# JunweiLiang/FVTA_MemexQA

Hardware: AMD Instinct MI355X
Metric: QA-pairs/sec (fwd+bwd) at B=64, 40 photos x 5 streams x 30 tok, h=512 (higher is better)
Workload: dtype bf16; 1 GPU; BASELINE.json configs[2] train step (fwd+bwd+adam), shape 'metric', dense lengths; qa_pairs_per_gpu=64, albums=1, photos=40, text_streams=5, hidden=512, global_batch=64, K=6, T=1200, JQ=30, parallelism=dp1 (QA pairs sharded, flat-gradient all-reduce)

## Files before the change

### fvta_memexqa_amd/csrc/lstm.hip

```cpp
#include "gemm_f32.h"
#include "fvta_prof.h"
#include <vector>

#include "lstm_common.h"

namespace fvta {

__device__ const float k_ones4[4] = {1.f, 0.f, 0.f, 0.f};


__global__ __launch_bounds__(1024) void plan_sort_kernel(PlanView v, const int32_t* __restrict__ len_in,
                                                         const int32_t* __restrict__ seq_J_in,
                                                         const int64_t* __restrict__ x_off_in,
                                                         const int64_t* __restrict__ out_off_in,
                                                         int64_t out_ld, int B, int J, int in, int d,
                                                         int64_t x_bw_delta) {
  extern __shared__ int32_t sh[];
  const int tid = threadIdx.x, wave = tid >> 6, lane = tid & 63;
  const int NW = 16, H = J + 1;
  for (int i = tid; i < NW * H; i += 1024) sh[i] = 0;
  const bool fresh = v.hdr->magic != PLAN_MAGIC || v.hdr->B != B || v.hdr->J != J || v.hdr->d != d || v.hdr->out_ld != out_ld;
  __syncthreads();
  if (tid == 0) {
    v.hdr->out_ld = out_ld;
// ... 599 lines not shown
  fvta_prof_end(FVTA_PROF_LSTM_STEP_FWD + 16 * d->reserved, launches, stream);
  FVTA_CHECK_LAUNCH("lstm_step_fwd");
  return FVTA_OK;
}

extern "C" int fvta_bilstm_bwd(const fvta_lstm_desc* d, const void* plan, const float* x, const float* out,
                               const float* d_out, const float* kernel_fw, const float* kernel_bw, void* saved,
                               float* dx, float* dkernel_fw, float* dbias_fw, float* dkernel_bw,
                               float* dbias_bw, void* workspace, fvta_stream_t stream_) {
  return fvta_bilstm_bwd_hint(d, plan, x, out, d_out, kernel_fw, kernel_bw, saved, dx, dkernel_fw, dbias_fw, dkernel_bw,
                              dbias_bw, workspace, stream_, nullptr, nullptr);
}

extern "C" int fvta_bilstm_bwd_overlap(const fvta_lstm_desc* d, const void* plan, const float* x, const float* out,
                                       const float* d_out, const float* kernel_fw, const float* kernel_bw, void* saved,
                                       float* dx, float* dkernel_fw, float* dbias_fw, float* dkernel_bw,
                                       float* dbias_bw, void* workspace, fvta_stream_t stream_,
                                       fvta_stream_t side_stream_) {
  return fvta_bilstm_bwd_hint(d, plan, x, out, d_out, kernel_fw, kernel_bw, saved, dx, dkernel_fw, dbias_fw, dkernel_bw,
                              dbias_bw, workspace, stream_, side_stream_, nullptr);
}

extern "C" int fvta_bilstm_bwd_hint(const fvta_lstm_desc* d, const void* plan, const float* x, const float* out,
                                    const float* d_out, const float* kernel_fw, const float* kernel_bw, void* saved,
                                    float* dx, float* dkernel_fw, float* dbias_fw, float* dkernel_bw,
                                    float* dbias_bw, void* workspace, fvta_stream_t stream_,
                                    fvta_stream_t side_stream_, const int32_t* nactive_host) {
  if (int e = check_lstm_desc(d)) return e;
  FVTA_CHECK_ARG(d->training, "bilstm_bwd: forward was not run with training=1");
  FVTA_CHECK_ARG(plan && x && out && d_out && kernel_fw && saved && dkernel_fw && dbias_fw && workspace,
                 "bilstm_bwd: null pointer");
  FVTA_CHECK_ARG(d->share_fw_bw || (kernel_bw && dkernel_bw && dbias_bw), "bilstm_bwd: *_bw pointers required");
  hipStream_t stream = (hipStream_t)stream_;
  PlanView pv = plan_view(d, const_cast<void*>(plan));
  SavedView sv = saved_view(d, saved);
  WorkView wv = work_view(d, workspace);
  const int B = d->B, J = d->J, in = d->in, dd = d->d;
  if (!lstm_is_bf(d)) FVTA_CHECK_HIP(hipMemsetAsync(wv.cstate, 0, (size_t)2 * B * dd * sizeof(float) * 2, stream));
  GateBwdArgs g;
  g.plan = pv;
  g.d_out = d_out;
  g.gates = sv.gates;
  g.gatesb = sv.gatesb;
  g.cs = sv.cs;
  g.dc = wv.cstate;
  g.dh_rec = wv.dh_rec;
  const bool bf = lstm_is_bf(d);
  g.dzb = bf ? wv.dzb : nullptr;
  g.B = B;
  g.J = J;
  g.d = dd;
  StepBwdArgs s;
  s.plan = pv;
  s.dz = sv.gates;
  s.W[0] = kernel_fw;
  s.W[1] = d->share_fw_bw ? kernel_fw : kernel_bw;
  s.dx = dx;
  s.dh_rec = wv.dh_rec;
  s.dzb = wv.dzb;
  s.in_i = in_internal(d);
  const int dbg = fvta_diag_env("FVTA_DEBUG_SKIP", 0);
  s.dbg = dbg;
  s.Wb[0] = wv.wb[0];
  s.Wb[1] = d->share_fw_bw ? wv.wb[0] : wv.wb[1];
  s.B = B;
  s.J = J;
  s.in = in;
  s.d = dd;
  const dim3 ggrid((unsigned)(((size_t)B * dd + 255) / 256), 1, 2);
  const dim3 sgrid((B + MmaSq::BM - 1) / MmaSq::BM, (in + dd + MmaSq::BN - 1) / MmaSq::BN, 2);
  const size_t sh = MmaSq::LDS_FLOATS * sizeof(float);
  DwArgs w;
  w.plan = pv;
  w.x = x;
  w.out = out;
  w.dz = sv.gates;
  w.slabs = wv.slabs;
  w.B = B;
  w.J = J;
  w.in = in;
  w.d = dd;
  w.tgroup = dw_tgroup(d);
  w.nsplit = dw_nsplit(d);
  w.dzb = wv.dzb;
  w.in_i = in_internal(d);
  w.xs = sv.xs;
  w.hs = sv.hs;
  w.xm = lstm_xm(d);
  (void)side_stream_;
  fvta_prof_begin(FVTA_PROF_LSTM_STEP_BWD + 16 * d->reserved, stream);
  if (bf) {
    FusedBwdArgs f;
    f.plan = pv;
    f.Wb[0] = wv.wb[0];
    f.Wb[1] = d->share_fw_bw ? wv.wb[0] : wv.wb[1];
    f.gatesb = sv.gatesb;
    f.cs = sv.cs;
    f.d_out = d_out;
    f.dzb = wv.dzb;
    f.dc = wv.cstate;
    f.dx = dx;
    f.B = B;
    f.J = J;
    f.in = in;
    f.d = dd;
    f.in_i = in_internal(d);
    f.gates32 = sv.gates;
    f.xm = lstm_xm(d);
    f.dx_accumulate = 1;
    f.dx_both = 0;
    if (dx && d->dx_overwrite) {
      const bool direct = dx_writes_whole_rows(f);
      hipLaunchKernelGGL(dx_zero_rows_kernel, dim3((B + 3) / 4), dim3(256), 0, stream, pv, dx, in, direct ? 1 : 0, B);
      f.dx_accumulate = direct ? 0 : 1;
    }
    for (int t = J - 1; t >= 0; --t) {
      f.t = t;
      f.nact_hint = nactive_host ? nactive_host[t] : -1;
      launch_bwd_fused_bf16(f, stream);
    }
    fvta_prof_end(FVTA_PROF_LSTM_STEP_BWD + 16 * d->reserved, J, stream);
    if (dx) {
      fvta_prof_begin(FVTA_PROF_LSTM_DX + 16 * d->reserved, stream);
      launch_dx_bf16(f, stream);
      fvta_prof_end(FVTA_PROF_LSTM_DX + 16 * d->reserved, 1, stream);
    }
  } else {
  if (dx && d->dx_overwrite) hipLaunchKernelGGL(dx_zero_rows_kernel, dim3((B + 3) / 4), dim3(256), 0, stream, pv, dx, in, 0, B);
  for (int t = J - 1; t >= 0; --t) {
    g.t = t;
    s.t = t;
    if (!(dbg & 512)) hipLaunchKernelGGL(lstm_gate_bwd, ggrid, dim3(256), 0, stream, g);
    if (t > 0 || dx) hipLaunchKernelGGL(lstm_step_bwd_f32, sgrid, dim3(256), sh, stream, s);
  }
  }
  if (!bf) fvta_prof_end(FVTA_PROF_LSTM_STEP_BWD + 16 * d->reserved, 2 * J, stream);
  FVTA_CHECK_LAUNCH("lstm_step_bwd");
  const int MM = in + dd + 1, N4 = 4 * dd;
  const dim3 wgrid((MM + MmaSq::BM - 1) / MmaSq::BM, N4 / MmaSq::BN, 2 * w.nsplit);
  fvta_prof_begin(FVTA_PROF_LSTM_DW + 16 * d->reserved, stream);
  if (dbg & 1024) {
  } else if (bf)
    launch_dw_bf16(w, stream);
  else
    hipLaunchKernelGGL(lstm_dw_f32, wgrid, dim3(256), sh, stream, w);
  FVTA_CHECK_LAUNCH("lstm_dw");
  const size_t slab_elems = bf ? (size_t)kpad8(d) * N4 : (size_t)MM * N4;
  const unsigned rgrid = (unsigned)((slab_elems + 255) / 256);
  if (bf) {
    const int ndir = d->share_fw_bw ? 1 : 2;
    for (int i = 0; i < ndir; ++i)
      launch_dw_reduce_bf16(wv.slabs + (size_t)i * w.nsplit * slab_elems, d->share_fw_bw ? 2 * w.nsplit : w.nsplit,
                            in, in_internal(d), dd, i == 0 ? dkernel_fw : dkernel_bw, i == 0 ? dbias_fw : dbias_bw,
                            stream);
  } else if (d->share_fw_bw) {
    hipLaunchKernelGGL(lstm_dw_reduce, dim3(rgrid), dim3(256), 0, stream, wv.slabs, 2 * w.nsplit, slab_elems,
                       in + dd, N4, dkernel_fw, dbias_fw);
  } else {
    hipLaunchKernelGGL(lstm_dw_reduce, dim3(rgrid), dim3(256), 0, stream, wv.slabs, w.nsplit, slab_elems, in + dd,
                       N4, dkernel_fw, dbias_fw);
    hipLaunchKernelGGL(lstm_dw_reduce, dim3(rgrid), dim3(256), 0, stream, wv.slabs + (size_t)w.nsplit * slab_elems,
                       w.nsplit, slab_elems, in + dd, N4, dkernel_bw, dbias_bw);
  }
  fvta_prof_end(FVTA_PROF_LSTM_DW + 16 * d->reserved, 1, stream);
  FVTA_CHECK_LAUNCH("lstm_dw_reduce");
  return FVTA_OK;
// ... 98 lines not shown
```

### fvta_memexqa_amd/csrc/lstm_bf16.hip

```cpp
#include "gemm_bf16.h"
#include "lstm_common.h"

namespace fvta {

__device__ __forceinline__ int il32(int e) { return ((e >> 5) << 6) + (e & 31); }
__global__ void cvt_weights_kernel(const float* __restrict__ W, bf16_t* __restrict__ wt, bf16_t* __restrict__ wb,
                                   int in, int in_i, int d, int xm) {
  __shared__ float tile[32][33];
  const int N4 = 4 * d, Ki = in_i + d;
  const int k0 = blockIdx.y * 32, n0 = blockIdx.x * 32;
  const int tx = threadIdx.x & 31, ty = threadIdx.x >> 5;
  for (int r = ty; r < 32; r += 8) {
    const int k = k0 + r, n = n0 + tx;
    const int src = k < in ? k : (k >= in_i ? in + (k - in_i) : -1);
    const float v = src >= 0 ? W[(size_t)src * N4 + n] : 0.f;
    tile[r][tx] = v;
    const int c = 4 * (n % d) + n / d;
    const bf16_t hi = f2bf(v);
    bf16_t* row = wb + (size_t)k * N4 * xm;
    if (xm == 1) {
      row[c] = hi;
    } else {
      row[il32(c)] = hi;
      row[il32(c) + 32] = f2bf(v - bf2f(hi));
// ... 462 lines not shown
        }
      }
#pragma unroll
      for (int it = 0; it < 4; ++it) {
        const f32x4 v = old[it] + plane_row16(pl, it * 8 + io_row, io_c4);
        if (ok[it] && (!(abl & 4) || v[0] == 1234.5f)) {
          if ((reinterpret_cast<uintptr_t>(ptr[it]) & 15) == 0) {
            *reinterpret_cast<f32x4*>(ptr[it]) = v;
          } else {
            ptr[it][0] = v[0]; ptr[it][1] = v[1]; ptr[it][2] = v[2]; ptr[it][3] = v[3];
          }
        }
      }
      wave_sync();
    }
}

#ifndef FVTA_DX_WIDE
#define FVTA_DX_WIDE 1
#endif
#ifndef FVTA_DX_BOTH
#define FVTA_DX_BOTH 1
#endif
static bool dx_wide_both(const FusedBwdArgs& a) {
  return FVTA_DX_WIDE && FVTA_DX_BOTH && a.in > 128 && a.in <= 256 && (4 * a.d * a.xm) % 64 == 0 &&
         (size_t)a.J * a.B * (4 * a.d * a.xm) * 2 < ((size_t)1 << 32);
}
bool dx_writes_whole_rows(const FusedBwdArgs& a) { return dx_wide_both(a); }

template <int WN, int BK, int ST, bool BOTH, bool NOACC, int XM, int WM = 4, int TN = 4>
static void launch_dx_tile(const FusedBwdArgs& a, dim3 grid, int dir, int accumulate, hipStream_t s) {
  typedef TileCfgT<WN, 2, WM, ST, BK, TN> Cfg;
  auto* k = lstm_dx_bf16<WN, BK, ST, BOTH, NOACC, XM, WM, TN>;
  lstm_launch(k, grid, dim3(Cfg::NT), Cfg::LDS_BYTES + Cfg::BM * 8, s, a, dir, accumulate);
}

template <int XM>
static void launch_dx_xm(const FusedBwdArgs& a, hipStream_t s) {
  if (FVTA_DX_WIDE && a.in > 128 && a.in <= 256 && (4 * a.d * a.xm) % 64 == 0) {
#ifndef FVTA_DX_BK
#define FVTA_DX_BK 64
#define FVTA_DX_ST 2
#endif
    static_assert(XM == 1 || FVTA_DX_BK == 64, "split engine: 64-element stage rows");
    constexpr int BK = FVTA_DX_BK, ST = FVTA_DX_ST;
    const dim3 grid(pad8((a.B + 255) / 256), 1, a.J);
    if (dx_wide_both(a)) {
      FusedBwdArgs b = a;
      b.dx_both = 1;
      if (!a.dx_accumulate)
        launch_dx_tile<2, BK, ST, true, true, XM>(b, grid, 0, 0, s);
      else
        launch_dx_tile<2, BK, ST, true, false, XM>(b, grid, 0, a.dx_accumulate, s);
      launch_dx_tile<2, BK, ST, false, false, XM>(b, grid, 1, a.dx_accumulate, s);
      return;
    }
    for (int dir = 0; dir < 2; ++dir) launch_dx_tile<2, BK, ST, false, false, XM>(a, grid, dir, a.dx_accumulate || dir, s);
    return;
  }
  constexpr int NBK = XM == 1 ? 32 : 64, NST = XM == 1 ? 3 : 2;
  if (XM == 2 && a.B <= 64 && a.in <= 128) {
    const dim3 gridp((a.B + 63) / 64, 1, a.J);
    for (int dir = 0; dir < 2; ++dir) launch_dx_tile<4, NBK, NST, false, false, XM, 1, 1>(a, gridp, dir, a.dx_accumulate || dir, s);
    return;
  }
  const dim3 grid(pad8((a.B + 255) / 256), (a.in + 127) / 128, a.J);
  for (int dir = 0; dir < 2; ++dir) launch_dx_tile<1, NBK, NST, false, false, XM>(a, grid, dir, a.dx_accumulate || dir, s);
}

void launch_dx_bf16(const FusedBwdArgs& a, hipStream_t s) {
  if (a.xm == 2)
    launch_dx_xm<2>(a, s);
  else
    launch_dx_xm<1>(a, s);
}

#ifndef FVTA_DW_STAGES
#define FVTA_DW_STAGES 4
#endif
constexpr int dw_stages(int wn) { return wn == 2 ? FVTA_DW_STAGES : 3; }
template <int WN>
using DwCfg = TileCfgT<WN, 2, 4, dw_stages(WN)>;

template <int WN>
__global__ __launch_bounds__((TileCfgT<WN>::NT), (WN == 1 ? 2 : 1)) void lstm_dw_bf16(DwArgs a) {
  typedef DwCfg<WN> TileCfg;
  typedef MmaBT<WN, 2, 4, dw_stages(WN)> MmaB;
  extern __shared__ __attribute__((aligned(16))) bf16_t smem_h[];
  const int tid = threadIdx.x;
  const int d = a.d, in_i = a.in_i, N4 = 4 * d;
  const int xtiles = (in_i + TileCfg::BM - 1) / TileCfg::BM;
  const int mtiles = xtiles + (d + TileCfg::BM - 1) / TileCfg::BM, ntiles = N4 / TileCfg::BN, per = mtiles * ntiles;
  const int xcd = blockIdx.x & 7, slot = blockIdx.x >> 3;
  const int bz = xcd + 8 * (slot / per);
  const int tile_id = slot % per;
  if (bz >= 2 * a.nsplit) return;
  const int bx = tile_id % mtiles, by = tile_id / mtiles;
  const bool isx = bx < xtiles;
  const int col0 = isx ? bx * TileCfg::BM : (bx - xtiles) * TileCfg::BM;
  const int ncols = isx ? in_i : d;
  const int n0 = by * TileCfg::BN;
  const int split = bz % a.nsplit, dir = bz / a.nsplit;
  MmaB mma;
  mma.init(tid);
  KMajorSrc<TileCfg::BM, TileCfg::A_GLDS> sa;
  KMajorSrc<TileCfg::BN, TileCfg::B_GLDS> sb;
  sa.setup(mma.wave_all, mma.lane, col0, ncols, (unsigned)ncols * 2);
  sb.setup(mma.wave_all, mma.lane, n0, N4, (unsigned)N4 * 2);
  const int t_begin = split * a.tgroup, t_end = min(a.J, t_begin + a.tgroup);
  for (int t = t_begin; t < t_end; ++t) {
    const int nact = a.plan.nactive[t];
    if (nact == 0) break;
    if (!isx && t == 0) continue;
    const size_t trow = ((size_t)dir * a.J + t) * a.B;
    const bf16_t* A = isx ? a.xs + trow * in_i : a.hs + (trow - (size_t)a.B) * d;
    const __amdgpu_buffer_rsrc_t ra = make_rsrc(A, (unsigned)nact * ncols * 2);
    const __amdgpu_buffer_rsrc_t rz = make_rsrc(a.dzb + trow * (size_t)N4, (unsigned)nact * N4 * 2);
    auto issue = [&](int tile, bf16_t* As, bf16_t* Bs) {
      sa.issue(ra, As, mma.wave_all, (unsigned)tile * 32u * ncols * 2u);
      sb.issue(rz, Bs, mma.wave_all, (unsigned)tile * 32u * N4 * 2u);
    };
    glds_mainloop<true>(mma, issue, (nact + 31) / 32, smem_h);
    __builtin_amdgcn_s_barrier();
  }
  float* slab = a.slabs + (size_t)bz * (in_i + d) * N4;
  const int mrow0 = isx ? col0 : in_i + col0;
#pragma unroll
  for (int ti = 0; ti < MmaB::TM; ++ti)
#pragma unroll
    for (int r = 0; r < 16; ++r) {
      const int ml = mma.row_of(ti, r);
      if (col0 + ml >= ncols) continue;
#pragma unroll
      for (int tj = 0; tj < MmaB::TN; ++tj) slab[(size_t)(mrow0 + ml) * N4 + n0 + mma.col_of(tj)] = mma.acc[ti][tj][r];
    }
}

__global__ __launch_bounds__(512, 1) void lstm_dw_x2(DwArgs a) {
  typedef DwX2Cfg TileCfg;
  extern __shared__ __attribute__((aligned(16))) bf16_t smem_h[];
  const int tid = threadIdx.x;
  const int d = a.d, in_i = a.in_i, N4 = 4 * d;
  const int xtiles = (in_i + TileCfg::BM - 1) / TileCfg::BM;
  const int mtiles = xtiles + (d + TileCfg::BM - 1) / TileCfg::BM, ntiles = (N4 + TileCfg::BN - 1) / TileCfg::BN, per = mtiles * ntiles;
  const int xcd = blockIdx.x & 7, slot = blockIdx.x >> 3;
  const int bz = xcd + 8 * (slot / per);
  const int tile_id = slot % per;
  if (bz >= 2 * a.nsplit) return;
  const int bx = tile_id % mtiles, by = tile_id / mtiles;
  const bool isx = bx < xtiles;
  const int col0 = isx ? bx * TileCfg::BM : (bx - xtiles) * TileCfg::BM;
  const int ncols = isx ? in_i : d;
  const int n0 = by * TileCfg::BN;
  const int split = bz % a.nsplit, dir = bz / a.nsplit;
  MmaX2K mma;
  mma.init(tid);
  KMajorSrc<TileCfg::PCOLS, TileCfg::A_GLDS> sa;
  KMajorSrc<TileCfg::PCOLS, TileCfg::B_GLDS> sb;
  sa.setup(mma.wave_all, mma.lane, 2 * col0, 2 * ncols, (unsigned)ncols * 4);
  sb.setup(mma.wave_all, mma.lane, 2 * n0, 2 * N4, (unsigned)N4 * 4);
  const int t_begin = split * a.tgroup, t_end = min(a.J, t_begin + a.tgroup);
  for (int t = t_begin; t < t_end; ++t) {
    const int nact = a.plan.nactive[t];
    if (nact == 0) break;
    if (!isx && t == 0) continue;
    const size_t trow = ((size_t)dir * a.J + t) * a.B;
    const bf16_t* A = isx ? a.xs + trow * (size_t)(2 * in_i) : a.hs + (trow - (size_t)a.B) * (size_t)(2 * d);
    const __amdgpu_buffer_rsrc_t ra = make_rsrc(A, (unsigned)nact * ncols * 4);
    const __amdgpu_buffer_rsrc_t rz = make_rsrc(a.dzb + trow * (size_t)(2 * N4), (unsigned)nact * N4 * 4);
    auto issue = [&](int tile, bf16_t* As, bf16_t* Bs) {
      sa.issue(ra, As, mma.wave_all, (unsigned)tile * TileCfg::KR * ncols * 4u);
      sb.issue(rz, Bs, mma.wave_all, (unsigned)tile * TileCfg::KR * N4 * 4u);
    };
    glds_mainloop<true>(mma, issue, (nact + TileCfg::KR - 1) / TileCfg::KR, smem_h);
    __builtin_amdgcn_s_barrier();
  }
  float* slab = a.slabs + (size_t)bz * (in_i + d) * N4;
  const int mrow0 = isx ? col0 : in_i + col0;
#pragma unroll
  for (int ti = 0; ti < MmaX2K::TM; ++ti)
#pragma unroll
    for (int r = 0; r < 16; ++r) {
      const int ml = mma.row_of(ti, r);
      if (col0 + ml >= ncols) continue;
#pragma unroll
      for (int tj = 0; tj < MmaX2K::TN; ++tj)
        if (n0 + mma.col_of(tj) < N4) slab[(size_t)(mrow0 + ml) * N4 + n0 + mma.col_of(tj)] = mma.acc[ti][tj][r];
    }
}

template <class Cfg, class K>
static void launch_dw_tiles(K* k, const DwArgs& a, hipStream_t s) {
  const int slices8 = (2 * a.nsplit + 7) / 8;
  const int per = ((a.in_i + 255) / 256 + (a.d + 255) / 256) * ((4 * a.d + Cfg::BN - 1) / Cfg::BN);
  lstm_launch(k, dim3(8 * per * slices8), dim3(Cfg::NT), Cfg::LDS_BYTES, s, a);
}
void launch_dw_bf16(const DwArgs& a, hipStream_t s) {
  if (a.xm == 2)
    launch_dw_tiles<DwX2Cfg>(lstm_dw_x2, a, s);
  else if ((4 * a.d) % 256 == 0)
    launch_dw_tiles<DwCfg<2>>(lstm_dw_bf16<2>, a, s);
  else
    launch_dw_tiles<DwCfg<1>>(lstm_dw_bf16<1>, a, s);
}

__global__ __launch_bounds__(256) void lstm_dw_reduce_bf16(const float* __restrict__ slabs, int nslab, int in, int in_i, int d,
                                                            float* __restrict__ dW, float* __restrict__ dbias) {
  const int N4 = 4 * d;
  const size_t slab_elems = (size_t)(in_i + d) * N4;
  const size_t idx = ((size_t)blockIdx.x * blockDim.x + threadIdx.x) * 4;
  if (idx >= slab_elems) return;
  const int row = (int)(idx / N4), u = (int)(idx % N4) >> 2;
  if (row > in && row < in_i) return;
  f32x4 s = f32x4{0.f, 0.f, 0.f, 0.f};
  int k = 0;
  for (; k + 8 <= nslab; k += 8) {
    f32x4 v[8];
#pragma unroll
    for (int j = 0; j < 8; ++j) v[j] = *reinterpret_cast<const f32x4*>(slabs + (size_t)(k + j) * slab_elems + idx);
#pragma unroll
    for (int j = 0; j < 8; ++j) s += v[j];
  }
  for (; k < nslab; ++k) s += *reinterpret_cast<const f32x4*>(slabs + (size_t)k * slab_elems + idx);
  float* dst = row < in ? dW + (size_t)row * N4 : (row == in ? dbias : dW + (size_t)(in + row - in_i) * N4);
#pragma unroll
  for (int g = 0; g < 4; ++g) dst[g * d + u] += s[g];
}

void launch_dw_reduce_bf16(const float* slabs, int nslab, int in, int in_i, int d, float* dW, float* dbias,
                           hipStream_t s) {
  const size_t n = (size_t)(in_i + d) * d;
  lstm_launch(lstm_dw_reduce_bf16, dim3((unsigned)((n + 255) / 256)), dim3(256), 0, s, slabs, nslab, in, in_i, d, dW, dbias);
}

__global__ void cvt_f32_bf16_kernel(const float* __restrict__ src, bf16_t* __restrict__ dst, size_t n) {
  const size_t i = (size_t)blockIdx.x * blockDim.x + threadIdx.x;
  if (i < n) dst[i] = f2bf(src[i]);
}

template <int LAYOUT>
__global__ __launch_bounds__(256, 2) void test_gemm_bf16_kernel(int M, int N, int K, const bf16_t* __restrict__ A,
                                                                const bf16_t* __restrict__ B, float* __restrict__ C) {
  extern __shared__ __attribute__((aligned(16))) bf16_t smem_h[];
  const int tid = threadIdx.x;
  const int m0 = blockIdx.x * TileCfg::BM, n0 = blockIdx.y * TileCfg::BN;
  MmaB mma;
  mma.init(tid);
  if (LAYOUT == 1) {
    const __amdgpu_buffer_rsrc_t ra = make_rsrc(A, (unsigned)M * K * 2), rb = make_rsrc(B, (unsigned)N * K * 2);
    RowSrc<TileCfg::A_GLDS> sa;
    RowSrc<TileCfg::B_GLDS> sb;
    sa.setup(mma.wave, mma.lane, m0, M, K * 2);
    sb.setup(mma.wave, mma.lane, n0, N, K * 2);
    auto issue = [&](int tile, bf16_t* As, bf16_t* Bs) {
      sa.issue(ra, As, mma.wave, tile * 64);
      sb.issue(rb, Bs, mma.wave, tile * 64);
    };
    glds_mainloop_sp(mma, issue, K / 32, smem_h);
  } else {
    const __amdgpu_buffer_rsrc_t ra = make_rsrc(A, (unsigned)K * M * 2), rb = make_rsrc(B, (unsigned)K * N * 2);
    KMajorSrc<TileCfg::BM, TileCfg::A_GLDS> sa;
    KMajorSrc<TileCfg::BN, TileCfg::B_GLDS> sb;
    sa.setup(mma.wave, mma.lane, m0, M, (unsigned)M * 2);
    sb.setup(mma.wave, mma.lane, n0, N, (unsigned)N * 2);
    auto issue = [&](int tile, bf16_t* As, bf16_t* Bs) {
      sa.issue(ra, As, mma.wave, (unsigned)tile * 32u * M * 2u);
      sb.issue(rb, Bs, mma.wave, (unsigned)tile * 32u * N * 2u);
    };
    glds_mainloop<true>(mma, issue, (K + 31) / 32, smem_h);
  }
#pragma unroll
  for (int ti = 0; ti < MmaB::TM; ++ti)
#pragma unroll
    for (int r = 0; r < 16; ++r) {
      const int m = m0 + mma.row_of(ti, r);
#pragma unroll
      for (int tj = 0; tj < MmaB::TN; ++tj) {
        const int n = n0 + mma.col_of(tj);
        if (m < M && n < N) C[(size_t)m * N + n] = mma.acc[ti][tj][r];
// ... 112 lines not shown
```

### fvta_memexqa_amd/csrc/lstm_common.h

```cpp
#pragma once
#include <type_traits>
#include "fvta_common.h"

namespace fvta {

struct PlanHeader {
  int64_t out_ld;
  int32_t B, J, in, d;
  int64_t x_bw_delta;
  uint32_t magic;
  int32_t pad[7];
};
constexpr uint32_t PLAN_MAGIC = 0x46565441u;

struct PlanView {
  PlanHeader* hdr;
  int32_t* order;
  int32_t* nactive;
  int32_t* len;
  int32_t* seq_J;
  int64_t* x_off;
  int64_t* out_off;
  int64_t* xo;
  int64_t* oo;
  int32_t* dirty;
  int64_t* dirty_out;
  size_t bytes;
};

static inline PlanView plan_view(const fvta_lstm_desc* d, void* p) {
  FvtaCarver c(p);
  PlanView v;
  v.hdr = c.take<PlanHeader>(1);
  v.order = c.take<int32_t>(d->B);
  v.nactive = c.take<int32_t>(d->J + 1);
  v.len = c.take<int32_t>(d->B);
  v.seq_J = c.take<int32_t>(d->B);
  v.x_off = c.take<int64_t>(d->B);
  v.out_off = c.take<int64_t>(d->B);
  v.xo = c.take<int64_t>((size_t)2 * d->J * d->B);
  v.oo = c.take<int64_t>((size_t)2 * d->J * d->B);
  v.dirty = c.take<int32_t>(d->B);
  v.dirty_out = c.take<int64_t>(d->B);
  v.bytes = c.off;
  return v;
}

static inline bool lstm_is_bf(const fvta_lstm_desc* d) { return d->precision == FVTA_BF16 || d->precision == FVTA_BF16X3; }
static inline int lstm_xm(const fvta_lstm_desc* d) { return d->precision == FVTA_BF16X3 ? 2 : 1; }

static inline int in_internal(const fvta_lstm_desc* d) { return (d->in + 1 + 31) / 32 * 32; }

struct SavedView {
  float* gates;
  bf16_t* gatesb;
  float* cs;
  bf16_t* xs;
  bf16_t* hs;
  size_t bytes;
};
static inline SavedView saved_view(const fvta_lstm_desc* d, void* p) {
  FvtaCarver c(p);
  SavedView s;
  s.gates = s.cs = nullptr;
  s.xs = s.hs = s.gatesb = nullptr;
  if (d->training) {
    if (d->precision == FVTA_BF16)
      s.gatesb = c.take<bf16_t>((size_t)2 * d->J * d->B * 4 * d->d);
    else
      s.gates = c.take<float>((size_t)2 * d->J * d->B * 4 * d->d);
    s.cs = c.take<float>((size_t)2 * d->J * d->B * d->d);
  }
  if (lstm_is_bf(d)) {
    s.xs = c.take<bf16_t>((size_t)2 * d->J * d->B * in_internal(d) * lstm_xm(d));
    s.hs = c.take<bf16_t>((size_t)2 * d->J * d->B * d->d * lstm_xm(d));
  }
  s.bytes = c.off < 256 ? 256 : c.off;
  return s;
}

static inline int dw_tgroup(const fvta_lstm_desc* d) {
  int g = (d->J + 15) / 16;
  return g < 1 ? 1 : g;
}
static inline int dw_nsplit(const fvta_lstm_desc* d) { return (d->J + dw_tgroup(d) - 1) / dw_tgroup(d); }
static inline int kpad8(const fvta_lstm_desc* d) { return in_internal(d) + d->d; }

struct WorkView {
  float* cstate;
  float* dh_rec;
  float* slabs;
  bf16_t* wt[2];
  bf16_t* wb[2];
  bf16_t* dzb;
  bf16_t* wf[2];
  size_t bytes;
};
static inline WorkView work_view(const fvta_lstm_desc* d, void* p) {
  FvtaCarver c(p);
  WorkView w;
  w.cstate = c.take<float>((size_t)2 * d->B * d->d);
  w.dh_rec = c.take<float>((size_t)2 * d->B * d->d);
  const size_t slab_rows = lstm_is_bf(d) ? (size_t)kpad8(d) : (size_t)(d->in + d->d + 1);
  w.slabs = c.take<float>((size_t)2 * dw_nsplit(d) * slab_rows * 4 * d->d);
  w.wt[0] = w.wt[1] = w.wb[0] = w.wb[1] = nullptr;
  w.dzb = nullptr;
  w.wf[0] = w.wf[1] = nullptr;
  if (lstm_is_bf(d)) {
    const size_t xm = (size_t)lstm_xm(d);
    for (int i = 0; i < 2; ++i) {
      w.wt[i] = c.take<bf16_t>((size_t)4 * d->d * kpad8(d) * xm);
      w.wb[i] = c.take<bf16_t>((size_t)kpad8(d) * 4 * d->d * xm);
    }
    if (d->training) w.dzb = c.take<bf16_t>((size_t)2 * d->J * d->B * 4 * d->d * xm);
    for (int i = 0; i < 2; ++i) w.wf[i] = c.take<bf16_t>((size_t)4 * d->d * kpad8(d) * xm);
  }
  w.bytes = c.off;
  return w;
}

struct StepArgs {
  PlanView plan;
  const float* x;
  float* out;
  const float* W[2];
  const bf16_t* Wt[2];
  const bf16_t* Wf[2];
  const bf16_t* xs;
  bf16_t* hs;
  const float* bias[2];
  float* gates;
  bf16_t* gatesb;
  float* cs;
  float* cstate;
  int t, B, J, in, d, Kp;
  int dbg;
  int xm;
  int nt;
  int64_t out_skip;
};

struct GateBwdArgs {
  PlanView plan;
  const float* d_out;
  float* gates;
  const bf16_t* gatesb;
  bf16_t* dzb;
  const float* cs;
  float* dc;
  float* dh_rec;
  int t, B, J, d;
};

struct StepBwdArgs {
  PlanView plan;
  const float* dz;
  const bf16_t* dzb;
  const float* W[2];
  const bf16_t* Wb[2];
  float* dx;
  float* dh_rec;
  int t, B, J, in, d, in_i;
  int dbg;
};

struct DwArgs {
  PlanView plan;
  const float* x;
  const float* out;
  const float* dz;
  const bf16_t* dzb;
  const bf16_t* xs;
  const bf16_t* hs;
  float* slabs;
  int B, J, in, d, tgroup, nsplit, in_i;
  int xm;
};

#ifdef __HIPCC__
template <class Mma>
__device__ __forceinline__ void lstm_gate_epilogue(const Mma& mma, const StepArgs& a, int dir, int m0, int u0,
                                                   int nact, size_t trow, const int64_t* s_oo) {
  static_assert(Mma::TN == 4 && Mma::WAVES_N == 1, "wave tile must span the four gate strips");
  const int d = a.d, t = a.t;
  const float* __restrict__ bias = a.bias[dir];
  const int u = u0 + mma.l31;
  const float bi = bias[u], bj = bias[d + u], bf = bias[2 * d + u], bo = bias[3 * d + u];
  const float* cprev_src = a.cs ? a.cs + (trow - a.B) * (size_t)d : a.cstate + (size_t)dir * a.B * d;
#pragma unroll
  for (int ti = 0; ti < Mma::TM; ++ti) {
    float cp[16];
#pragma unroll
    for (int r = 0; r < 16; ++r) {
      const int i = min(m0 + mma.row_of(ti, r), nact - 1);
      cp[r] = (t > 0 && !(a.dbg & 64)) ? cprev_src[(size_t)i * d + u] : 0.f;
    }
#pragma unroll
    for (int r = 0; r < 16; ++r) {
      const int row = mma.row_of(ti, r);
      const int i = m0 + row;
      const float ig = fvta_sigmoid(mma.acc[ti][0][r] + bi);
      const float jg = fvta_tanh(mma.acc[ti][1][r] + bj);
      const float fg = fvta_sigmoid(mma.acc[ti][2][r] + bf + 1.0f);
      const float og = fvta_sigmoid(mma.acc[ti][3][r] + bo);
      const float c = cp[r] * fg + ig * jg;
      const float h = fvta_tanh(c) * og;
      if (i < nact) {
        if (a.cs) {
          if (!(a.dbg & 16)) a.cs[(trow + i) * d + u] = c;
          if (a.dbg & 8) {
          } else if (a.gatesb) {
            bf16x4 pk;
            pk[0] = (short)f2bf(ig);
            pk[1] = (short)f2bf(jg);
            pk[2] = (short)f2bf(fg);
            pk[3] = (short)f2bf(og);
            *reinterpret_cast<bf16x4*>(a.gatesb + (trow + i) * (size_t)(4 * d) + 4 * u) = pk;
          } else {
            float* g = a.gates + (trow + i) * (size_t)(4 * d) + u;
            g[0] = ig;
            g[d] = jg;
            g[2 * d] = fg;
            g[3 * d] = og;
          }
        } else {
          a.cstate[((size_t)dir * a.B + i) * d + u] = c;
        }
        if (!(a.dbg & 4) && s_oo[row] >= a.out_skip) a.out[s_oo[row] + u] = h;
        if (a.hs && !(a.dbg & 32)) a.hs[(trow + i) * d + u] = f2bf(h);
      }
    }
  }
}
#endif

#ifdef __HIPCC__
template <int B, int E, class F>
__device__ __forceinline__ void static_for(F&& f) {
  if constexpr (B < E) {
    f(std::integral_constant<int, B>{});
    static_for<B + 1, E>(f);
  }
}

__device__ __forceinline__ unsigned pk_bf16(float a, float b) {
  typedef __bf16 bf16x2_t __attribute__((ext_vector_type(2)));
  typedef float f32x2_t __attribute__((ext_vector_type(2)));
  return __builtin_bit_cast(unsigned, __builtin_convertvector(f32x2_t{a, b}, bf16x2_t));
}

__device__ __forceinline__ void wave_sync() {
  asm volatile("s_waitcnt lgkmcnt(0)" ::: "memory");
  __builtin_amdgcn_wave_barrier();
}

__device__ __forceinline__ void st16(float* p, const f32x4 v, bool nt) {
  if (nt)
    __builtin_nontemporal_store(v, reinterpret_cast<f32x4*>(p));
  else
// ... 82 lines not shown
        const int i = m0 + wrow0 + (r & 3) + 8 * (r >> 2) + 4 * mma.hf;
        if (i < nact) *reinterpret_cast<f32x4*>(a.gates + (trow + i) * (size_t)(4 * d) + 4 * u) = f32x4{ig, jg, fg, og};
      }
    }
    {
#pragma unroll
      for (int r = 0; r < 16; ++r) pl[plane_c_idx(r, mma.hf, mma.l31)] = cv[r];
      wave_sync();
      float* dst = a.cs ? a.cs + trow * d : a.cstate + (size_t)dir * a.B * d;
#pragma unroll
      for (int it = 0; it < 4; ++it) {
        const int lr = it * 8 + io_row, i = m0 + wrow0 + lr;
        const f32x4 v = plane_row16(pl, lr, io_c4);
        if (i < nact) st16(dst + (size_t)i * d + u0 + 4 * io_c4, v, a.nt != 0);
      }
      wave_sync();
    }
    {
#pragma unroll
      for (int r = 0; r < 16; ++r) pl[plane_c_idx(r, mma.hf, mma.l31)] = hv[r];
      wave_sync();
#pragma unroll
      for (int it = 0; it < 4; ++it) {
        const int lr = it * 8 + io_row;
        const int64_t oo = s_oo[wrow0 + lr];
        const f32x4 v = plane_row16(pl, lr, io_c4);
        if (oo >= a.out_skip) {
          float* o = a.out + oo + u0 + 4 * io_c4;
          if ((reinterpret_cast<uintptr_t>(o) & 15) == 0) {
            st16(o, v, a.nt != 0);
          } else {
            o[0] = v[0]; o[1] = v[1]; o[2] = v[2]; o[3] = v[3];
          }
        }
      }
      wave_sync();
    }
    if (a.hs) {
      constexpr int LDH = 40;
      const size_t hld = (size_t)d * a.xm;
#pragma unroll
      for (int term = 0; term < 2; ++term) {
        if (term >= a.xm) break;
        const bool lo = term == 1;
#pragma unroll
        for (int r = 0; r < 16; ++r) {
          const bf16_t hi = f2bf(hv[r]);
          plh[((r & 3) + 8 * (r >> 2) + 4 * mma.hf) * LDH + mma.l31] = lo ? f2bf(hv[r] - bf2f(hi)) : hi;
        }
        wave_sync();
#pragma unroll
        for (int it = 0; it < 2; ++it) {
          const int lr = it * 16 + (lane >> 2), c8 = lane & 3, i = m0 + wrow0 + lr;
          const f32x4 v = *reinterpret_cast<const f32x4*>(&plh[lr * LDH + 8 * c8]);
          if (i < nact) *reinterpret_cast<f32x4*>(a.hs + (trow + i) * hld + (size_t)a.xm * u0 + 32 * term + 8 * c8) = v;
        }
        wave_sync();
      }
    }
    if (a.gatesb) {
      constexpr int LDG = 136;
#pragma unroll
      for (int r = 0; r < 16; ++r)
        *reinterpret_cast<bf16x4*>(&plh[((r & 3) + 8 * (r >> 2) + 4 * mma.hf) * LDG + 4 * mma.l31]) = gv[r];
      wave_sync();
#pragma unroll
      for (int it = 0; it < 8; ++it) {
        const int lr = it * 4 + (lane >> 4), c8 = lane & 15, i = m0 + wrow0 + lr;
        const f32x4 v = *reinterpret_cast<const f32x4*>(&plh[lr * LDG + 8 * c8]);
        if (i < nact) st16(reinterpret_cast<float*>(a.gatesb + (trow + i) * (size_t)(4 * d) + 4 * u0 + 8 * c8), v, a.nt != 0);
      }
      wave_sync();
    }
  }
}

#endif

void launch_cvt_weights_bf16(const float* W, bf16_t* wt, bf16_t* wb, int in, int in_i, int d, int xm, hipStream_t s);
void launch_cvt_x_bf16(const PlanView& pv, const float* x, bf16_t* xs, int B, int J, int in, int in_i, int xm, hipStream_t s);
void launch_step_fwd_bf16(const StepArgs& a, hipStream_t s);
int wreg_nct(int in_i, int d);
int wreg_mode();
bool wreg_x3_built(int in_i, int d);
void launch_cvt_weights_frag(const float* W, const float* bias, bf16_t* wf, int in, int in_i, int d, int xm, hipStream_t s);
bool launch_step_fwd_wreg(const StepArgs& a, hipStream_t s);
struct FusedBwdArgs {
  PlanView plan;
  const bf16_t* Wb[2];
  const bf16_t* gatesb;
  const float* cs;
  const float* d_out;
  bf16_t* dzb;
  float* dc;
  float* dx;
  int t, B, J, in, d, in_i;
  int nact_hint;
  const float* gates32;
  int xm;
  int dx_accumulate;
  int dx_both;
};
void launch_bwd_fused_bf16(const FusedBwdArgs& a, hipStream_t s);
bool launch_bwd_wreg(const FusedBwdArgs& a, hipStream_t s);
void launch_dx_bf16(const FusedBwdArgs& a, hipStream_t s);
bool dx_writes_whole_rows(const FusedBwdArgs& a);
void launch_dw_bf16(const DwArgs& a, hipStream_t s);
void launch_dw_reduce_bf16(const float* slabs, int nslab, int in, int in_i, int d, float* dW, float* dbias, hipStream_t s);
int test_gemm_bf16(int layout, int M, int N, int K, const float* A, const float* B, float* C, hipStream_t s);

}
```

### fvta_memexqa_amd/csrc/lstm_wreg.hip

```cpp
#include "gemm_bf16.h"
#include "lstm_common.h"

namespace fvta {

template <int NX16_, int ND16_, int NCT_, bool X3_ = false>
struct WregCfg {
  static constexpr int NX16 = NX16_, ND16 = ND16_, NCT = NCT_, NW = 4;
  static constexpr bool X3 = X3_;
  static_assert(!X3_ || NCT_ == 1, "split engine: one column tile per wave (its hi and lo fragments fill the register file)");
  static constexpr int NWF = X3 ? 2 : NCT;
  static constexpr int NP = X3 ? 3 : NCT;
  static constexpr int NACC = X3 ? 2 : NCT;
  static constexpr int KS = X3 ? 4 : 8;
  static constexpr int NK16 = NX16 + ND16;
  static constexpr int NU = 8 * NCT, UB = NW * NU;
  static constexpr int RW = 32 / NW, DP = 8 / NW;
  static constexpr int D = 16 * ND16, IN_I = 16 * NX16;
  static constexpr int XM = X3 ? 2 : 1;
  static constexpr int CB = D / UB;
  static constexpr int SX = (NX16 + KS - 1) / KS, SH = ND16 / KS, S = SX + SH;
  static constexpr int XLAST = NX16 - KS * (SX - 1);
  static constexpr int RT = S >= 12 ? 1 : 12 / S, RING = RT * S, LOOK = RING - 2;
  static constexpr int SLOT_ELEMS = 32 * 128;
  static constexpr int TILE_ELEMS = S * SLOT_ELEMS;
// ... 359 lines not shown
        const unsigned long long r0 = WREG_CLOCK();
        own_rows(m0);
        st_rows += WREG_CLOCK() - r0;
      }
      static_for<0, C::NP>([&](auto pl_c) {
        constexpr int pl = decltype(pl_c)::value;
        if constexpr (C::X3 && pl == 2)
          mfma(q_c, pl_c, frl[C::buf_of(q)].b);
        else
          mfma(q_c, pl_c, fr[C::buf_of(q)].b);
        if constexpr (C::stage_begin(C::NP * q + pl) < C::stage_begin(C::NP * q + pl + 1)) {
          const unsigned long long g0 = WREG_CLOCK();
          if constexpr (!(abl & 1)) static_for<C::stage_begin(C::NP * q + pl), C::stage_begin(C::NP * q + pl + 1)>([&](auto s_c) { run_stage(s_c, prev_m0); });
          st_stage += WREG_CLOCK() - g0;
        }
      });
      }
    };
    static_for<0, C::NV>([&](auto q_c) {
      kstep(q_c);
      constexpr int q1 = decltype(q_c)::value + 1;
      if constexpr (q1 < C::NK16) {
#pragma unroll
        for (int ct = 0; ct < NWF; ++ct)
          if (q1 * NWF + ct >= C::W_REG_FRAGS) wl[ct].f = wlds[(q1 * NWF + ct - C::W_REG_FRAGS) * 64];
      }
    });
    const unsigned long long sl0 = WREG_CLOCK();
    if constexpr (!C::SLAB_SAFE) {
      asm volatile("s_waitcnt lgkmcnt(0)" ::: "memory");
      __builtin_amdgcn_s_barrier();
      asm volatile("" ::: "memory");
    }
    if constexpr (C::NACC > 1)
      asm volatile("s_nop 15\n\ts_nop 3" : "+a"(acc[0]), "+a"(acc[C::NACC - 1]));
    else
      asm volatile("s_nop 15\n\ts_nop 3" : "+a"(acc[0]));
    if constexpr (!(abl & 64)) {
    if constexpr (C::X3) {
      float* zc = zs + (l31 / C::NU) * C::UB + wave * C::NU + l31 % C::NU;
#pragma unroll
      for (int r = 0; r < 16; ++r) zc[((r & 3) + 8 * (r >> 2) + 4 * hf) * C::ZS] = acc[0][r] + acc[1][r];
    } else {
#pragma unroll
    for (int ct = 0; ct < NCT; ++ct) {
      const int idx = ct * 32 + l31;
      float* zc = zs + (idx / C::NU) * C::UB + wave * C::NU + idx % C::NU;
#pragma unroll
      for (int r = 0; r < 16; ++r) zc[((r & 3) + 8 * (r >> 2) + 4 * hf) * C::ZS] = acc[ct][r];
    }
    }
    }
    st_slab += WREG_CLOCK() - sl0;
    prev_m0 = m0;
#pragma unroll
    for (int p = 0; p < C::PASSES; ++p) {
      cp_cur[p] = cp_next[p];
      oo_cur[p] = oo_next[p];
    }
#pragma unroll
    for (int ks = 0; ks < C::KS; ++ks) {
      ap[ks] += tb_delta;
      if constexpr (C::X3) apl[ks] += tb_delta;
    }
  }
  asm volatile("s_waitcnt lgkmcnt(0)" ::: "memory");
  __builtin_amdgcn_s_barrier();
  asm volatile("" ::: "memory");
  static_for<0, C::NSTAGES>([&](auto s_c) { run_stage(s_c, prev_m0); });
  wait_vmcnt<0>();
#ifdef FVTA_WREG_STAMP
  if (t == 5 && (int)blockIdx.x == a.dbg && tid == 0) {
    g_wreg_stamps[0] = st_t0; g_wreg_stamps[1] = st_t1; g_wreg_stamps[2] = WREG_CLOCK(); g_wreg_stamps[3] = nmine;
    g_wreg_stamps[4] = st_wait; g_wreg_stamps[5] = st_bar; g_wreg_stamps[6] = st_slab; g_wreg_stamps[7] = st_n;
    g_wreg_stamps[8] = st_issue; g_wreg_stamps[9] = st_stage; g_wreg_stamps[10] = st_rows;
  }
#endif
}

static int g_wreg_override = -1;
int wreg_mode() {
  static const int env_mode = [] {
    const char* e = getenv("FVTA_LSTM_WREG");
    return (e && e[0] >= '0' && e[0] <= '7') ? e[0] - '0' : 7;
  }();
  return g_wreg_override >= 0 ? g_wreg_override : env_mode;
}
int wreg_set_mode(int mode) {
  const int prev = wreg_mode();
  g_wreg_override = mode < 0 ? -1 : (mode & 7);
  return prev;
}

template <class F>
static bool wreg_visit(int in_i, int d, bool x3, F&& f) {
  if (!(wreg_mode() & 1) || in_i % 16 || d % 128) return false;
  auto row = [&](auto c) {
    typedef decltype(c) C;
    if (C::IN_I != in_i || C::D != d || C::X3 != x3) return false;
    f(c);
    return true;
  };
  return row(WregCfg<14, 32, 2>{}) || row(WregCfg<8, 32, 2>{}) || row(WregCfg<14, 64, 1>{}) || row(WregCfg<8, 64, 1>{}) ||
         row(WregCfg<8, 8, 2>{}) || row(WregCfg<2, 8, 2>{}) ||
         row(WregCfg<14, 32, 1, true>{}) || row(WregCfg<8, 32, 1, true>{}) || row(WregCfg<8, 8, 1, true>{}) || row(WregCfg<2, 8, 1, true>{});
}

int wreg_nct(int in_i, int d) {
  int nct = 0;
  wreg_visit(in_i, d, false, [&](auto c) { nct = decltype(c)::NCT; });
  return nct;
}
bool wreg_x3_built(int in_i, int d) { return wreg_visit(in_i, d, true, [](auto) {}); }

void launch_cvt_weights_frag(const float* W, const float* bias, bf16_t* wf, int in, int in_i, int d, int xm, hipStream_t s) {
  wreg_visit(in_i, d, xm == 2, [&](auto c) {
    typedef decltype(c) C;
    const int nk16 = (in_i + d) / 16;
    const size_t total = (size_t)d * nk16 * 8 * C::XM;
    auto* k = cvt_weights_frag_kernel<C::X3 ? 2 : C::NCT, C::X3>;
    lstm_launch(k, dim3((unsigned)((total + 255) / 256)), dim3(256), 0, s, W, bias, wf, in, in_i, d, nk16);
  });
}

bool launch_step_fwd_wreg(const StepArgs& a, hipStream_t s) {
  if (!a.Wf[0] || !a.hs) return false;
  return wreg_visit(a.Kp - a.d, a.d, a.xm == 2, [&](auto c) {
    typedef decltype(c) C;
    auto* k = lstm_fwd_wreg_bf16<C>;
    const int rg = wreg_row_groups(C::CB, (a.B + 31) / 32);
    lstm_launch(k, dim3(2 * rg * C::CB), dim3(64 * C::NW), C::LDS_BYTES, s, a, rg);
  });
}

}
```

Baseline: 5431 QA-pairs/s.

## Balance LSTM weight-gradient split-K work across fixed slices of active row tiles

The LSTM backward dW kernels previously split work by groups of timesteps, which gives uneven loads when the number of active rows varies across time. They now count the total row tiles over all timesteps and give each of 16 fixed slices an equal contiguous range, so every block does about the same K-work. This aims to cut tail imbalance and raise occupancy in the dW reduction. The cost is more slab memory (16 slices per direction) and a larger slab reduction, plus a per-block prefix count over nactive. It is on by default and can be disabled through an environment variable.

```diff
diff --git a/fvta_memexqa_amd/csrc/lstm.hip b/fvta_memexqa_amd/csrc/lstm.hip
--- a/fvta_memexqa_amd/csrc/lstm.hip
+++ b/fvta_memexqa_amd/csrc/lstm.hip
@@ -705,6 +705,8 @@
   w.d = dd;
   w.tgroup = dw_tgroup(d);
   w.nsplit = dw_nsplit(d);
+  w.kslices = lstm_is_bf(d) && dw_kslices_on();
+  if (w.kslices) w.nsplit = DW_KSLICES;
   w.dzb = wv.dzb;
   w.in_i = in_internal(d);
   w.xs = sv.xs;
diff --git a/fvta_memexqa_amd/csrc/lstm_bf16.hip b/fvta_memexqa_amd/csrc/lstm_bf16.hip
--- a/fvta_memexqa_amd/csrc/lstm_bf16.hip
+++ b/fvta_memexqa_amd/csrc/lstm_bf16.hip
@@ -568,6 +568,39 @@
 template <int WN>
 using DwCfg = TileCfgT<WN, 2, 4, dw_stages(WN)>;
 
+template <class Cfg, class K>
+static void launch_dw_tiles(K* k, const DwArgs& a, hipStream_t s) {
+  const int slices8 = (2 * a.nsplit + 7) / 8;
+  const int per = ((a.in_i + 255) / 256 + (a.d + 255) / 256) * ((4 * a.d + Cfg::BN - 1) / Cfg::BN);
+  lstm_launch(k, dim3(8 * per * slices8), dim3(Cfg::NT), Cfg::LDS_BYTES, s, a);
+}
+template <int KT, class Step>
+__device__ __forceinline__ void dw_walk(const DwArgs& a, int split, bool isx, Step&& step) {
+  const int* __restrict__ nactive = a.plan.nactive;
+  if (!a.kslices) {
+    const int t_begin = split * a.tgroup, t_end = min(a.J, t_begin + a.tgroup);
+    for (int t = t_begin; t < t_end; ++t) {
+      const int nact = nactive[t];
+      if (nact == 0) break;
+      if (!isx && t == 0) continue;
+      step(t, nact, 0, (nact + KT - 1) / KT);
+    }
+    return;
+  }
+  const int t0 = isx ? 0 : 1;
+  int total = 0;
+#pragma unroll 8
+  for (int t = t0; t < a.J; ++t) total += (nactive[t] + KT - 1) / KT;
+  const int k_lo = (int)((long long)total * split / a.nsplit), k_hi = (int)((long long)total * (split + 1) / a.nsplit);
+  int base = 0;
+  for (int t = t0; t < a.J && base < k_hi; ++t) {
+    const int nact = __builtin_amdgcn_readfirstlane(nactive[t]), n = (nact + KT - 1) / KT;
+    const int lo = max(k_lo - base, 0), hi = min(k_hi - base, n);
+    if (lo < hi) step(t, nact, lo, hi);
+    base += n;
+  }
+}
+
 template <int WN>
 __global__ __launch_bounds__((TileCfgT<WN>::NT), (WN == 1 ? 2 : 1)) void lstm_dw_bf16(DwArgs a) {
   typedef DwCfg<WN> TileCfg;
@@ -593,22 +626,18 @@
   KMajorSrc<TileCfg::BN, TileCfg::B_GLDS> sb;
   sa.setup(mma.wave_all, mma.lane, col0, ncols, (unsigned)ncols * 2);
   sb.setup(mma.wave_all, mma.lane, n0, N4, (unsigned)N4 * 2);
-  const int t_begin = split * a.tgroup, t_end = min(a.J, t_begin + a.tgroup);
-  for (int t = t_begin; t < t_end; ++t) {
-    const int nact = a.plan.nactive[t];
-    if (nact == 0) break;
-    if (!isx && t == 0) continue;
+  dw_walk<32>(a, split, isx, [&](int t, int nact, int lo, int hi) {
     const size_t trow = ((size_t)dir * a.J + t) * a.B;
     const bf16_t* A = isx ? a.xs + trow * in_i : a.hs + (trow - (size_t)a.B) * d;
     const __amdgpu_buffer_rsrc_t ra = make_rsrc(A, (unsigned)nact * ncols * 2);
     const __amdgpu_buffer_rsrc_t rz = make_rsrc(a.dzb + trow * (size_t)N4, (unsigned)nact * N4 * 2);
     auto issue = [&](int tile, bf16_t* As, bf16_t* Bs) {
-      sa.issue(ra, As, mma.wave_all, (unsigned)tile * 32u * ncols * 2u);
-      sb.issue(rz, Bs, mma.wave_all, (unsigned)tile * 32u * N4 * 2u);
+      sa.issue(ra, As, mma.wave_all, (unsigned)(lo + tile) * 32u * ncols * 2u);
+      sb.issue(rz, Bs, mma.wave_all, (unsigned)(lo + tile) * 32u * N4 * 2u);
     };
-    glds_mainloop<true>(mma, issue, (nact + 31) / 32, smem_h);
+    glds_mainloop<true>(mma, issue, hi - lo, smem_h);
     __builtin_amdgcn_s_barrier();
-  }
+  });
   float* slab = a.slabs + (size_t)bz * (in_i + d) * N4;
   const int mrow0 = isx ? col0 : in_i + col0;
 #pragma unroll
@@ -645,22 +674,18 @@
   KMajorSrc<TileCfg::PCOLS, TileCfg::B_GLDS> sb;
   sa.setup(mma.wave_all, mma.lane, 2 * col0, 2 * ncols, (unsigned)ncols * 4);
   sb.setup(mma.wave_all, mma.lane, 2 * n0, 2 * N4, (unsigned)N4 * 4);
-  const int t_begin = split * a.tgroup, t_end = min(a.J, t_begin + a.tgroup);
-  for (int t = t_begin; t < t_end; ++t) {
-    const int nact = a.plan.nactive[t];
-    if (nact == 0) break;
-    if (!isx && t == 0) continue;
+  dw_walk<TileCfg::KR>(a, split, isx, [&](int t, int nact, int lo, int hi) {
     const size_t trow = ((size_t)dir * a.J + t) * a.B;
     const bf16_t* A = isx ? a.xs + trow * (size_t)(2 * in_i) : a.hs + (trow - (size_t)a.B) * (size_t)(2 * d);
     const __amdgpu_buffer_rsrc_t ra = make_rsrc(A, (unsigned)nact * ncols * 4);
     const __amdgpu_buffer_rsrc_t rz = make_rsrc(a.dzb + trow * (size_t)(2 * N4), (unsigned)nact * N4 * 4);
     auto issue = [&](int tile, bf16_t* As, bf16_t* Bs) {
-      sa.issue(ra, As, mma.wave_all, (unsigned)tile * TileCfg::KR * ncols * 4u);
-      sb.issue(rz, Bs, mma.wave_all, (unsigned)tile * TileCfg::KR * N4 * 4u);
+      sa.issue(ra, As, mma.wave_all, (unsigned)(lo + tile) * TileCfg::KR * ncols * 4u);
+      sb.issue(rz, Bs, mma.wave_all, (unsigned)(lo + tile) * TileCfg::KR * N4 * 4u);
     };
-    glds_mainloop<true>(mma, issue, (nact + TileCfg::KR - 1) / TileCfg::KR, smem_h);
+    glds_mainloop<true>(mma, issue, hi - lo, smem_h);
     __builtin_amdgcn_s_barrier();
-  }
+  });
   float* slab = a.slabs + (size_t)bz * (in_i + d) * N4;
   const int mrow0 = isx ? col0 : in_i + col0;
 #pragma unroll
@@ -675,12 +700,6 @@
     }
 }
 
-template <class Cfg, class K>
-static void launch_dw_tiles(K* k, const DwArgs& a, hipStream_t s) {
-  const int slices8 = (2 * a.nsplit + 7) / 8;
-  const int per = ((a.in_i + 255) / 256 + (a.d + 255) / 256) * ((4 * a.d + Cfg::BN - 1) / Cfg::BN);
-  lstm_launch(k, dim3(8 * per * slices8), dim3(Cfg::NT), Cfg::LDS_BYTES, s, a);
-}
 void launch_dw_bf16(const DwArgs& a, hipStream_t s) {
   if (a.xm == 2)
     launch_dw_tiles<DwX2Cfg>(lstm_dw_x2, a, s);
diff --git a/fvta_memexqa_amd/csrc/lstm_common.h b/fvta_memexqa_amd/csrc/lstm_common.h
--- a/fvta_memexqa_amd/csrc/lstm_common.h
+++ b/fvta_memexqa_amd/csrc/lstm_common.h
@@ -84,6 +84,7 @@
   return g < 1 ? 1 : g;
 }
 static inline int dw_nsplit(const fvta_lstm_desc* d) { return (d->J + dw_tgroup(d) - 1) / dw_tgroup(d); }
+constexpr int DW_KSLICES = 16;
 static inline int kpad8(const fvta_lstm_desc* d) { return in_internal(d) + d->d; }
 
 struct WorkView {
@@ -102,7 +103,8 @@
   w.cstate = c.take<float>((size_t)2 * d->B * d->d);
   w.dh_rec = c.take<float>((size_t)2 * d->B * d->d);
   const size_t slab_rows = lstm_is_bf(d) ? (size_t)kpad8(d) : (size_t)(d->in + d->d + 1);
-  w.slabs = c.take<float>((size_t)2 * dw_nsplit(d) * slab_rows * 4 * d->d);
+  const size_t nslab = lstm_is_bf(d) ? (size_t)2 * DW_KSLICES : (size_t)2 * dw_nsplit(d);
+  w.slabs = c.take<float>(nslab * slab_rows * 4 * d->d);
   w.wt[0] = w.wt[1] = w.wb[0] = w.wb[1] = nullptr;
   w.dzb = nullptr;
   w.wf[0] = w.wf[1] = nullptr;
@@ -175,6 +177,7 @@
   float* slabs;
   int B, J, in, d, tgroup, nsplit, in_i;
   int xm;
+  int kslices;
 };
 
 #ifdef __HIPCC__
@@ -423,6 +426,7 @@
 void launch_step_fwd_bf16(const StepArgs& a, hipStream_t s);
 int wreg_nct(int in_i, int d);
 int wreg_mode();
+bool dw_kslices_on();
 bool wreg_x3_built(int in_i, int d);
 void launch_cvt_weights_frag(const float* W, const float* bias, bf16_t* wf, int in, int in_i, int d, int xm, hipStream_t s);
 bool launch_step_fwd_wreg(const StepArgs& a, hipStream_t s);
diff --git a/fvta_memexqa_amd/csrc/lstm_wreg.hip b/fvta_memexqa_amd/csrc/lstm_wreg.hip
--- a/fvta_memexqa_amd/csrc/lstm_wreg.hip
+++ b/fvta_memexqa_amd/csrc/lstm_wreg.hip
@@ -465,13 +465,15 @@
 int wreg_mode() {
   static const int env_mode = [] {
     const char* e = getenv("FVTA_LSTM_WREG");
-    return (e && e[0] >= '0' && e[0] <= '7') ? e[0] - '0' : 7;
+    const char* k = getenv("FVTA_DW_KSLICES");
+    return ((e && e[0] >= '0' && e[0] <= '7') ? e[0] - '0' : 7) | ((k && k[0] == '0') ? 8 : 0);
   }();
   return g_wreg_override >= 0 ? g_wreg_override : env_mode;
 }
+bool dw_kslices_on() { return !(wreg_mode() & 8); }
 int wreg_set_mode(int mode) {
   const int prev = wreg_mode();
-  g_wreg_override = mode < 0 ? -1 : (mode & 7);
+  g_wreg_override = mode < 0 ? -1 : (mode & 15);
   return prev;
 }
 
```

After: 5355 QA-pairs/s. -1.4%, worse.
